# VIDILabs/instantvnr

Hardware: AMD Instinct MI355X
Metric: fps at 1024^2 on 1024^3 volume (higher is better)
Workload: dtype f16

## Files before the change

include/vnr_amd.h:

```cpp
#ifndef VNR_AMD_H
#define VNR_AMD_H

#include <stddef.h>
#include <stdint.h>

#ifdef __cplusplus
extern "C" {
#endif

#define VNR_AMD_OK 0
#define VNR_AMD_ERROR 1

typedef struct vnrAmdVolume_t*           vnrAmdVolume;
typedef struct vnrAmdRenderer_t*         vnrAmdRenderer;
typedef struct vnrAmdTransferFunction_t* vnrAmdTransferFunction;
typedef struct vnrAmdCamera_t*           vnrAmdCamera;

enum {
  VNR_AMD_OPTIX_NO_SHADING = 0,
  VNR_AMD_RAYMARCHING_NO_SHADING_DECODING = 4,
  VNR_AMD_RAYMARCHING_NO_SHADING_SAMPLE_STREAMING = 5,
  VNR_AMD_RAYMARCHING_NO_SHADING_IN_SHADER = 6,
  VNR_AMD_RAYMARCHING_GRADIENT_SHADING_SAMPLE_STREAMING = 8,
  VNR_AMD_RAYMARCHING_SINGLE_SHADE_HEURISTIC_SAMPLE_STREAMING = 11,
// ... 185 lines not shown
void vnrAmdReleaseVolume(vnrAmdVolume);

vnrAmdRenderer vnrAmdCreateRenderer(vnrAmdVolume);
int  vnrAmdRendererSetFramebufferSize(vnrAmdRenderer, int width, int height);
int  vnrAmdRendererSetTransferFunction(vnrAmdRenderer, vnrAmdTransferFunction);
int  vnrAmdRendererSetCamera(vnrAmdRenderer, vnrAmdCamera);
int  vnrAmdRendererSetMode(vnrAmdRenderer, int mode);
int  vnrAmdRendererSetDenoiser(vnrAmdRenderer, int enable);
int  vnrAmdRendererSetVolumeSamplingRate(vnrAmdRenderer, float rate);
int  vnrAmdRendererSetVolumeDensityScale(vnrAmdRenderer, float scale);
int  vnrAmdRendererResetAccumulation(vnrAmdRenderer);
int  vnrAmdRender(vnrAmdRenderer);
const float* vnrAmdRendererMapFrame(vnrAmdRenderer);
int  vnrAmdRendererSetOutputAsDeviceFramebuffer(vnrAmdRenderer, int enable);
int  vnrAmdRendererSetPixelRange(vnrAmdRenderer, uint32_t pixel_lo, uint32_t pixel_hi);
int  vnrAmdRendererSetPixelInterleave(vnrAmdRenderer, uint32_t block_pixels, uint32_t n_parts, uint32_t part);

typedef struct {
  uint64_t n_samples;
  uint64_t n_reference_slots;
  uint32_t n_iterations;
  uint32_t n_rays_hit;
  double   infer_kernel_ms;
  uint64_t infer_kernel_launches;
  double   infer_union_ms;
} vnrAmdFrameStats;
int  vnrAmdRendererGetFrameStats(vnrAmdRenderer, vnrAmdFrameStats*);
int  vnrAmdRendererSetProfiling(vnrAmdRenderer, int enable);
int  vnrAmdRendererSetAsync(vnrAmdRenderer, int enable);
int  vnrAmdRendererSetInShaderKernel(vnrAmdRenderer, int mode);
int  vnrAmdRendererDebugQueues(vnrAmdRenderer, const float** d_coords, const uint32_t** d_counters, float* iteration_ms, int max_iterations);
int  vnrAmdRendererDebugSchedule(vnrAmdRenderer, int out[4]);
int  vnrAmdDebugRaySourceIndex(const uint32_t* counts, uint32_t n_in, uint32_t* src_out, uint32_t* alive_out);
void vnrAmdReleaseRenderer(vnrAmdRenderer);

int  vnrAmdDistGetUniqueId(void* out128);
int  vnrAmdDistInit(int rank, int world_size, int local_rank, const void* unique_id, const char* transport, const char* address);
int  vnrAmdDistInitFromEnv(void);
int  vnrAmdDistFinalize(void);
int  vnrAmdDistRank(void);
int  vnrAmdDistWorldSize(void);
const char* vnrAmdDistTransport(void);
int  vnrAmdDistRcclRanksSeen(void);
int  vnrAmdDistBarrier(void);
int  vnrAmdDistAllReduceHost(double* values, int n, int op);
int  vnrAmdDistAllReduce(void* buf, size_t count, int dtype, int op);
int  vnrAmdDistAllGather(const void* send, void* recv, size_t bytes_per_rank);
int  vnrAmdDistReduceScatter(void* buf, size_t count_per_rank, int dtype);
int  vnrAmdDistBroadcast(void* buf, size_t bytes, int root);
int  vnrAmdDistSelfTest(double deadline_s, char* report, size_t report_size);
int  vnrAmdRendererSetDistributed(vnrAmdRenderer, int enable);
const float* vnrAmdRendererGatherFrame(vnrAmdRenderer);
int  vnrAmdRendererRenderPipelined(vnrAmdRenderer, const float** previous_frame);
int  vnrAmdRendererGetCompletedFrameStats(vnrAmdRenderer, vnrAmdFrameStats*);
int  vnrAmdRendererFlushPipeline(vnrAmdRenderer, const float** last_frame);
int  vnrAmdNeuralVolumeTrainDataParallel(vnrAmdVolume, int steps, int fast_mode);
int  vnrAmdNeuralVolumeSyncReplicas(vnrAmdVolume);
int  vnrAmdNeuralVolumeAllReduceGradients(vnrAmdVolume);
int  vnrAmdNeuralVolumeTrainEndDataParallel(vnrAmdVolume, int fast_mode, int sharded);
int  vnrAmdNeuralVolumeSetGradients(vnrAmdVolume, const float* host, size_t count);

int  vnrAmdMarchingCube(vnrAmdVolume, float isovalue, float** xyz, size_t* n_vertices, int on_device);
int  vnrAmdSaveTriangles(const char* filename, const float* xyz, size_t n_vertices);

void vnrAmdMemoryQuery(size_t* used_by_renderer, size_t* used_by_network);
void vnrAmdFreeTemporaryGPUMemory(void);
// ... 19 lines not shown
```

instantvnr_amd/_lib.py:

```python
import ctypes as C
import os
import re
import subprocess
import sys

_HERE = os.path.dirname(os.path.abspath(__file__))
ROOT = os.path.dirname(_HERE)
SO_PATH = os.environ.get("VNR_AMD_LIB_PATH") or os.path.join(_HERE, "libvnr_amd.so")
HEADER = os.path.join(ROOT, "include", "vnr_amd.h")

_lib = None
_torch_imported_before_load = None


class VnrAmdError(RuntimeError):
    pass


def require_torch_loaded_first():
    if _lib is not None and not _torch_imported_before_load:
        raise VnrAmdError("libvnr_amd.so was loaded before `import torch`: PyTorch's bundled ROCm runtime cannot share the "
                          "GPU with the system runtime the library already initialised.  Import torch first (instantvnr_amd."
                          "dist.init_from_env does when WORLD_SIZE > 1; tests/conftest.py does for the test session).")

# ... 148 lines not shown
    sig("vnrAmdNeuralVolumeSetInitSeed", I, P, U64)
    sig("vnrAmdVolumeSetClippingBox", I, P, FP, FP)
    sig("vnrAmdVolumeSetScaling", I, P, FP)
    sig("vnrAmdVolumeSetTransform", I, P, FP)
    sig("vnrAmdSimpleVolumeGetDataRange", I, P, FP)
    sig("vnrAmdMarchingCube", I, P, F, C.POINTER(C.POINTER(C.c_float)), C.POINTER(SZ), I)
    sig("vnrAmdSaveTriangles", I, C.c_char_p, C.POINTER(C.c_float), SZ)
    sig("vnrAmdVolumeGetValueRange", I, P, FP)
    sig("vnrAmdVolumeGetDims", I, P, IP)
    sig("vnrAmdVolumeIsNetwork", I, P)
    sig("vnrAmdVolumeGetMacrocell", I, P, IP, FP, C.POINTER(P), C.POINTER(P))
    sig("vnrAmdReleaseVolume", None, P)
    sig("vnrAmdCreateRenderer", P, P)
    sig("vnrAmdRendererSetFramebufferSize", I, P, I, I)
    sig("vnrAmdRendererSetTransferFunction", I, P, P)
    sig("vnrAmdRendererSetCamera", I, P, P)
    sig("vnrAmdRendererSetMode", I, P, I)
    sig("vnrAmdRendererSetDenoiser", I, P, I)
    sig("vnrAmdRendererSetVolumeSamplingRate", I, P, F)
    sig("vnrAmdRendererSetVolumeDensityScale", I, P, F)
    sig("vnrAmdRendererResetAccumulation", I, P)
    sig("vnrAmdRender", I, P)
    sig("vnrAmdRendererMapFrame", P, P)
    sig("vnrAmdRendererSetOutputAsDeviceFramebuffer", I, P, I)
    sig("vnrAmdRendererSetPixelRange", I, P, U32, U32)
    sig("vnrAmdRendererSetPixelInterleave", I, P, U32, U32, U32)
    sig("vnrAmdRendererGetFrameStats", I, P, C.POINTER(FrameStats))
    sig("vnrAmdRendererSetProfiling", I, P, I)
    sig("vnrAmdRendererSetAsync", I, P, I)
    sig("vnrAmdRendererSetInShaderKernel", I, P, I)
    sig("vnrAmdRendererDebugQueues", I, P, C.POINTER(P), C.POINTER(P), FP, I)
    sig("vnrAmdRendererDebugSchedule", I, P, IP)
    sig("vnrAmdDebugRaySourceIndex", I, P, U32, P, C.POINTER(U32))
    sig("vnrAmdReleaseRenderer", None, P)
    sig("vnrAmdDistGetUniqueId", I, P)
    sig("vnrAmdDistInit", I, I, I, I, P, C.c_char_p, C.c_char_p)
    sig("vnrAmdDistInitFromEnv", I)
    sig("vnrAmdDistFinalize", I)
    sig("vnrAmdDistRank", I)
    sig("vnrAmdDistWorldSize", I)
    sig("vnrAmdDistTransport", C.c_char_p)
    sig("vnrAmdDistRcclRanksSeen", I)
    sig("vnrAmdDistBarrier", I)
    sig("vnrAmdDistAllReduceHost", I, C.POINTER(D), I, I)
    sig("vnrAmdDistAllReduce", I, P, SZ, I, I)
    sig("vnrAmdDistAllGather", I, P, P, SZ)
    sig("vnrAmdDistReduceScatter", I, P, SZ, I)
    sig("vnrAmdDistBroadcast", I, P, SZ, I)
    sig("vnrAmdDistSelfTest", I, C.c_double, C.c_char_p, SZ)
    sig("vnrAmdRendererSetDistributed", I, P, I)
    sig("vnrAmdRendererGatherFrame", P, P)
    sig("vnrAmdRendererRenderPipelined", I, P, C.POINTER(P))
    sig("vnrAmdRendererGetCompletedFrameStats", I, P, C.POINTER(FrameStats))
    sig("vnrAmdRendererFlushPipeline", I, P, C.POINTER(P))
    sig("vnrAmdNeuralVolumeTrainDataParallel", I, P, I, I)
    sig("vnrAmdNeuralVolumeSyncReplicas", I, P)
    sig("vnrAmdNeuralVolumeSetBrickImageMode", I, P, I)
    sig("vnrAmdNeuralVolumeSetBrickImageBudget", I, P, SZ)
    sig("vnrAmdNeuralVolumeBrickImageLevels", C.c_uint, P)
    sig("vnrAmdNeuralVolumeGridBackwardPlan", I, P, U64, C.POINTER(U32), C.POINTER(U64))
    sig("vnrAmdNeuralVolumeSetDeterministicTraining", I, P, I)
    sig("vnrAmdNeuralVolumeGetDeterministicTraining", I, P, C.POINTER(I))
    sig("vnrAmdNeuralVolumeBrickImagePolicy", I, P, C.POINTER(U64), C.POINTER(C.c_uint), IP, C.POINTER(U64))
    sig("vnrAmdNeuralVolumeSetTrainProfiling", I, P, I)
    sig("vnrAmdNeuralVolumeGetTrainProfile", I, P, C.POINTER(D), IP)
    sig("vnrAmdNeuralVolumeAllReduceGradients", I, P)
# ... 57 lines not shown
```

instantvnr_amd/api.py:

```python
import ctypes as C
import json

import numpy as np

from . import _lib
from ._lib import VnrAmdError, check, check_ptr, lib

JSON_TEXT, JSON_BSON, JSON_TEXT_FILE, JSON_BSON_FILE = 0, 1, 2, 3

VALUE_TYPES = {np.dtype(np.uint8): 0, np.dtype(np.int8): 1, np.dtype(np.uint16): 2, np.dtype(np.int16): 3,
               np.dtype(np.uint32): 4, np.dtype(np.int32): 5, np.dtype(np.float32): 8, np.dtype(np.float64): 12}


def _fp(a):
    return a.ctypes.data_as(C.POINTER(C.c_float))


def _vec(v, n=3):
    a = np.ascontiguousarray(v, dtype=np.float32).ravel()
    assert a.size == n
    return a


def _json_arg(j, params=False):
# ... 708 lines not shown

def vnrRendererSetOutputAsDeviceFramebuffer(r, flag):
    check(lib().vnrAmdRendererSetOutputAsDeviceFramebuffer(r.h, 1 if flag else 0))
    r._device_output = bool(flag)


def vnrRendererSetProfiling(r, flag):
    check(lib().vnrAmdRendererSetProfiling(r.h, 1 if flag else 0))


def vnrRendererGetFrameStats(r):
    s = _lib.FrameStats()
    check(lib().vnrAmdRendererGetFrameStats(r.h, C.byref(s)))
    return {k: getattr(s, k) for k, _ in s._fields_}


def renderer_schedule(r):
    out = (C.c_int * 4)()
    check(lib().vnrAmdRendererDebugSchedule(r.h, out))
    return {"n_iters": out[0], "n_parts": out[1], "fused_pack": bool(out[2]), "decoupled": bool(out[3])}


def ray_source_index(counts, n_in):
    n_in = int(n_in)
    counts = np.ascontiguousarray(counts, dtype=np.uint32)
    if n_in <= 0 or counts.shape != ((n_in + 63) // 64,):
        raise ValueError("counts must hold one entry per 64-ray group of n_in > 0 rays")
    src = np.zeros(n_in, dtype=np.uint32)
    alive = C.c_uint32()
    check(lib().vnrAmdDebugRaySourceIndex(counts.ctypes.data, n_in, src.ctypes.data, C.byref(alive)))
    return src[:alive.value].copy(), int(alive.value)


def neural_brick_image(v):
    u, b, ms = C.c_int(), C.c_size_t(), C.c_float()
    check(lib().vnrAmdNeuralVolumeBrickImageInfo(v.h, C.byref(u), C.byref(b), C.byref(ms)))
    builds, after, tier, small = C.c_uint64(), C.c_uint(), C.c_int(), C.c_uint64()
    check(lib().vnrAmdNeuralVolumeBrickImagePolicy(v.h, C.byref(builds), C.byref(after), C.byref(tier), C.byref(small)))
    return {"in_use": bool(u.value), "bytes": b.value, "build_ms": ms.value, "levels": int(lib().vnrAmdNeuralVolumeBrickImageLevels(v.h)),
            "builds": int(builds.value), "launches_before_next_build": int(after.value), "tier": int(tier.value), "small_builds": int(small.value)}


def neural_set_brick_budget(v, n_bytes):
    check(lib().vnrAmdNeuralVolumeSetBrickImageBudget(v.h, int(n_bytes)))


def neural_info(v):
    vals = [C.c_int() for _ in range(5)]
    n = C.c_uint64()
    check(lib().vnrAmdNeuralVolumeGetInfo(v.h, *[C.byref(x) for x in vals], C.byref(n)))
    keys = ["n_levels", "n_features_per_level", "padded_width", "n_neurons", "n_hidden_layers"]
    d = {k: x.value for k, x in zip(keys, vals)}
    d["n_params"] = n.value
    kind = [C.c_int() for _ in range(6)]
    check(lib().vnrAmdNeuralVolumeGetModelKind(v.h, *[C.byref(x) for x in kind]))
    d.update({k: x.value for k, x in zip(["activation", "output_activation", "grid_type", "interpolation", "mfma_kernels", "mfma_training_kernels"], kind)})
    return d


def neural_grid_backward_plan(v, batch=65536):
    u32, u64 = (C.c_uint32 * 4)(), (C.c_uint64 * 2)()
    check(lib().vnrAmdNeuralVolumeGridBackwardPlan(v.h, int(batch), u32, u64))
    return {"n_levels": u32[0], "lds_levels": u32[1], "tile_entries": u32[2], "lds_blocks": u32[3], "atomic_requests": int(u64[0]), "flush_requests_at_most": int(u64[1])}


def neural_set_deterministic_training(v, enable=True):
# ... 183 lines not shown
```

instantvnr_amd/csrc/capi.cpp:

```cpp
#include "../../include/vnr_amd.h"

#include <cstdlib>
#include <cstdio>
#include <fstream>
#include <limits>
#include <memory>

#include "correction_budget.h"
#include "dist.h"
#include "renderer.h"
#include "scene.h"

using namespace vnr;

struct vnrAmdVolume_t { std::shared_ptr<VolumeBase> v; };
struct vnrAmdRenderer_t { std::unique_ptr<Renderer> r; std::shared_ptr<VolumeBase> volume; };
struct vnrAmdTransferFunction_t { TransferFunctionData d; };
struct vnrAmdCamera_t { CameraData d; };
struct vnrAmdCorrection_t { std::shared_ptr<Correction> c; };

namespace {
thread_local std::string g_last_error;

template <typename F>
// ... 988 lines not shown
}
int vnrAmdRendererGetFrameStats(vnrAmdRenderer r, vnrAmdFrameStats* s)
{
  return guarded([&]() {
    VNR_REN(r);
    const FrameStats& f = r->r->stats();
    s->n_samples = f.n_samples; s->n_reference_slots = f.n_reference_slots; s->n_iterations = f.n_iterations;
    s->n_rays_hit = f.n_rays_hit; s->infer_kernel_ms = f.infer_kernel_ms; s->infer_kernel_launches = f.infer_kernel_launches; s->infer_union_ms = f.infer_union_ms;
  });
}
int vnrAmdRendererDebugQueues(vnrAmdRenderer r, const float** d_coords, const uint32_t** d_counters, float* iteration_ms, int max_iterations)
{
  return guarded([&]() {
    VNR_REN(r);
    if (d_coords) *d_coords = r->r->debug_coords();
    if (d_counters) *d_counters = r->r->debug_counters();
    const auto& v = r->r->debug_iteration_ms();
    for (int i = 0; i < max_iterations; ++i) iteration_ms[i] = i < (int)v.size() ? v[i] : 0.0f;
  });
}
int vnrAmdRendererDebugSchedule(vnrAmdRenderer r, int out[4])
{
  return guarded([&]() {
    VNR_REN(r);
    if (!out) throw std::runtime_error("null output");
    const int* v = r->r->debug_schedule();
    for (int i = 0; i < 4; ++i) out[i] = v[i];
  });
}
int vnrAmdDebugRaySourceIndex(const uint32_t* counts, uint32_t n_in, uint32_t* src_out, uint32_t* alive_out)
{
  return guarded([&]() { debug_ray_source_index(counts, n_in, src_out, alive_out); });
}
int vnrAmdRendererSetProfiling(vnrAmdRenderer r, int e) { return guarded([&]() { VNR_REN(r); r->r->set_profiling(e != 0); }); }
int vnrAmdRendererSetAsync(vnrAmdRenderer r, int e) { return guarded([&]() { VNR_REN(r); r->r->set_async(e != 0); }); }
int vnrAmdRendererSetInShaderKernel(vnrAmdRenderer r, int m) { return guarded([&]() { VNR_REN(r); r->r->set_in_shader_kernel(m); }); }
void vnrAmdReleaseRenderer(vnrAmdRenderer r) { delete r; }

int vnrAmdDistGetUniqueId(void* out128) { return guarded([&]() { if (!out128) throw std::runtime_error("null id buffer"); rccl_unique_id(out128); }); }
static void bind_device_to_local_rank(int local_rank)
{
  const int count = vnrAmdDeviceCount();
  if (count > 0) Runtime::get().init(local_rank % count);
}
int vnrAmdDistInit(int rank, int world, int local_rank, const void* unique_id, const char* transport, const char* address)
{
  return guarded([&]() {
    bind_device_to_local_rank(local_rank);
    Dist::get().init(rank, world, local_rank, unique_id, transport, address ? address : "");
  });
}
int vnrAmdDistInitFromEnv(void)
{
  return guarded([&]() {
    const char* lr = std::getenv("LOCAL_RANK");
    const char* r = std::getenv("RANK");
    bind_device_to_local_rank(lr && *lr ? std::atoi(lr) : (r && *r ? std::atoi(r) : 0));
    Dist::get().init_from_env();
  });
}
int vnrAmdDistFinalize(void) { return guarded([&]() { Dist::get().finalize(); }); }
int vnrAmdDistRank(void) { return Dist::get().rank(); }
int vnrAmdDistWorldSize(void) { return Dist::get().world(); }
const char* vnrAmdDistTransport(void) { return Dist::get().transport_name(); }
int vnrAmdDistRcclRanksSeen(void) { return Dist::get().rccl_ranks_seen(); }
int vnrAmdDistBarrier(void)
// ... 220 lines not shown
```

instantvnr_amd/csrc/infer_kernel.h:

```cpp
#pragma once
#include <algorithm>
#include <cstdlib>

#include "infer_tile.h"
#include "pack_rays.h"

namespace vnr {

struct FusedMlp {
  const uint16_t* packed;
  uint32_t lds_halves, width, n_hidden_matmuls, activation, output_activation;
  bool general;
  bool weights_global;
  float quantize_threshold;
};

struct InferArgs {
  const LevelInfo* levels;
  uint32_t n_levels, interpolation;
  const half_t* table;
  uint32_t table_bytes;
  const uint8_t* brick_image;
  const half_t* packed_mlp;
  const float* coords;
  float* out;
  half_t* features_out;
  half_t* acts_out;
  const uint32_t* n_ptr;
  const uint32_t* dest;
  uint32_t queue_mode;
  uint32_t out_stride;
  uint32_t n;
  uint32_t n_hidden_matmuls;
  uint32_t activation;
  uint32_t output_activation;
  uint32_t lds_halves;
  uint32_t sharers;
  uint32_t weights_global;
  float quantize_threshold;
  PackArgs pack;
};

template <int F, int K_IN, int W, int MODE, bool GENERAL>
__global__ void __launch_bounds__(64 * MlpShape<W>::WAVES) fused_infer_kernel(const InferArgs args)
{
  constexpr int NCHUNK = K_IN / 8;
  constexpr uint32_t WAVES = MlpShape<W>::WAVES;
  extern __shared__ __attribute__((aligned(16))) half_t lds[];

  const uint32_t lane = threadIdx.x & 63u;
  const uint32_t wave = threadIdx.x >> 6;

  if (MODE == 0 && WAVES == 4 && args.pack.n_blocks) {
    uint32_t* s_part = (uint32_t*)lds;
    for (uint32_t item = blockIdx.x; item < args.pack.n_blocks; item += gridDim.x) {
      pack_rays_block<4>(args.pack, item, s_part);
      __syncthreads();
    }
  }
  const uint32_t n = args.n_ptr ? min(*args.n_ptr, args.n) : args.n;
  const uint32_t n_tiles = (n + 63u) >> 6;
  const uint32_t xcd = blockIdx.x & 7u;
  const uint32_t per_xcd = (n_tiles + 7u) >> 3;
  const uint32_t waves_per_xcd = (gridDim.x >> 3) * WAVES;
  const uint32_t tile_end = min(n_tiles, (xcd + 1u) * per_xcd);
  if (xcd * per_xcd + (blockIdx.x >> 3) * WAVES >= tile_end) return;

  constexpr bool CAN_GLOBAL = GENERAL;
  const bool wglobal = CAN_GLOBAL && args.weights_global != 0u;
  if (MODE != 1 && !wglobal) {
    const uint4_t* src = (const uint4_t*)args.packed_mlp;
    uint4_t* dst = (uint4_t*)lds;
    for (uint32_t i = threadIdx.x; i < args.lds_halves / 8; i += blockDim.x) dst[i] = src[i];
    __syncthreads();
  }
  const uint32_t nh = args.n_hidden_matmuls;
  const uint32_t act = args.activation;
  const uint32_t h = lane >> 5;
  const uint32_t r = lane & 31u;
  const table_rsrc_t rsrc = make_table_rsrc(args.table, args.table_bytes);

  for (uint32_t tile = xcd * per_xcd + (blockIdx.x >> 3) * WAVES + wave; tile < tile_end; tile += waves_per_xcd) {
    const uint32_t i = tile * 64u + lane;
    const uint32_t ic = min(i, n - 1u);
    float3_packed p;
    uint32_t out_index = i;
    if (args.queue_mode) {
      const uint4_t rec = ((const uint4_t*)args.coords)[ic];
      p = {__uint_as_float(rec.x), __uint_as_float(rec.y), __uint_as_float(rec.z)};
      out_index = rec.w * args.out_stride;
    } else {
      p = ((const float3_packed*)args.coords)[ic];
      if (args.dest) out_index = args.dest[ic];
    }

    half8_t feat[NCHUNK];
    encode_tile<F, K_IN, GENERAL>(args.levels, args.n_levels, args.interpolation, rsrc, args.brick_image, p.x, p.y, p.z, feat,
                                  GENERAL ? args.quantize_threshold : 0.0f);

    if (MODE != 0 && args.features_out && i < n) {
      half8_t* dst = (half8_t*)(args.features_out + (size_t)i * K_IN);
#pragma unroll
      for (int c = 0; c < NCHUNK; ++c) dst[c] = feat[c];
    }
    if (MODE == 1) continue;

    float y;
    if (CAN_GLOBAL && wglobal)
      y = mlp_tile<W, K_IN, MODE == 2, GENERAL>(args.packed_mlp, feat, nh, act, h, r, args.acts_out, n, tile * 64u);
    else
      y = mlp_tile<W, K_IN, MODE == 2, GENERAL>((const half_t*)lds, feat, nh, act, h, r, args.acts_out, n, tile * 64u);
    if (i < n) args.out[out_index] = finish_output<GENERAL>(y, args.output_activation);
  }
}

template <int F, int K_IN, int W, int MODE, bool GENERAL>
static void launch_one(const InferArgs& a, size_t n_max, hipStream_t s)
{
  constexpr uint32_t WAVES = MlpShape<W>::WAVES;
  const Runtime& rt = Runtime::get();
  const uint32_t n_tiles = div_round_up(n_max, 64);
  uint32_t blocks = div_round_up(n_tiles, WAVES);
  static const uint32_t forced = [] {
    const char* e = std::getenv("VNR_AMD_INFER_BLOCKS_PER_CU");
    const int v = e ? std::atoi(e) : 0;
    return (uint32_t)(v >= 1 && v <= 64 ? v : 0);
  }();
  const size_t shmem = (MODE == 1 || a.weights_global) ? 16 : (size_t)a.lds_halves * sizeof(uint16_t);
  const uint32_t fit = (uint32_t)std::max<size_t>(1, std::min<size_t>(4, (160 * 1024) / std::max<size_t>(shmem, 1)));
  uint32_t max_blocks = (uint32_t)rt.n_cus * (forced ? forced : std::min(fit, a.sharers >= 2 ? 3u : 4u));
  if (!forced && a.n_ptr && a.queue_mode) max_blocks = std::min((uint32_t)rt.n_cus * 32u, std::max((uint32_t)rt.n_cus * 4u, n_tiles / 33u));
  if (blocks > max_blocks) blocks = max_blocks;
  blocks = next_multiple(blocks, 8);
  auto kernel = fused_infer_kernel<F, K_IN, W, MODE, GENERAL>;
  static bool attr_set = false;
  if (!attr_set) {
    VNR_HIP_CHECK(hipFuncSetAttribute((const void*)kernel, hipFuncAttributeMaxDynamicSharedMemorySize, 160 * 1024));
    attr_set = true;
  }
  kernel<<<blocks, 64 * WAVES, shmem, s>>>(a);
  VNR_HIP_CHECK(hipGetLastError());
}

template <int W, int MODE, bool GENERAL>
static void dispatch(uint32_t F, uint32_t K_IN, const InferArgs& a, size_t n_max, hipStream_t s)
{
#define VNR_CASE(f, k) if (F == f && K_IN == k) return launch_one<f, k, W, MODE, GENERAL>(a, n_max, s)
  VNR_CASE(1, 16); VNR_CASE(1, 32);
  VNR_CASE(2, 16); VNR_CASE(2, 32); VNR_CASE(2, 48); VNR_CASE(2, 64);
  VNR_CASE(4, 16); VNR_CASE(4, 32); VNR_CASE(4, 48); VNR_CASE(4, 64); VNR_CASE(4, 80); VNR_CASE(4, 96); VNR_CASE(4, 112); VNR_CASE(4, 128);
  VNR_CASE(8, 16); VNR_CASE(8, 32); VNR_CASE(8, 48); VNR_CASE(8, 64); VNR_CASE(8, 80); VNR_CASE(8, 96); VNR_CASE(8, 112); VNR_CASE(8, 128);
#undef VNR_CASE
  throw std::runtime_error("unsupported encoding shape: n_features_per_level=" + std::to_string(F) +
                           " padded width=" + std::to_string(K_IN));
}

#define VNR_DEFINE_FUSED_WIDTH(W, GENERAL, SUFFIX)                                                                        \
  void launch_fused_w##W##SUFFIX(int mode, uint32_t F, uint32_t K_IN, const InferArgs& a, size_t n_max, hipStream_t s)    \
  {                                                                                                                       \
    if (mode == 0) dispatch<W, 0, GENERAL>(F, K_IN, a, n_max, s);                                                         \
    else dispatch<W, 2, GENERAL>(F, K_IN, a, n_max, s);                                                                   \
  }

}
```

instantvnr_amd/csrc/infer_tile.h:

```cpp
#pragma once
#include "grid_device.h"

namespace vnr {

struct float3_packed { float x, y, z; };

template <int W> struct MlpShape {
  static_assert(W == 16 || W == 32 || W == 64 || W == 128, "FullyFusedMLP widths");
  static constexpr int MT = W >= 32 ? W / 32 : 1;
  static constexpr int RW = 32 * MT;
  static constexpr int KS = W / 16;
  static constexpr int STEP = 16 * RW;
  static constexpr int HIDDEN = KS * STEP;
  static constexpr int LAST = KS * 16;
  static constexpr int WAVES = W == 128 ? 8 : 4;
};
__host__ __device__ inline uint32_t mlp_rows_padded(uint32_t W) { return W >= 32u ? W : 32u; }
__host__ __device__ inline uint32_t packed_mlp_halves(uint32_t in_width, uint32_t W, uint32_t n_hidden_matmuls)
{
  const uint32_t step = 16u * mlp_rows_padded(W);
  return (in_width / 16u) * step + n_hidden_matmuls * (W / 16u) * step + (W / 16u) * 16u;
}

__host__ __device__ inline uint32_t packedT_halves(uint32_t in_width, uint32_t W, uint32_t nh)
// ... 99 lines not shown
    for (int e = 0; e < 16; ++e) acc[m][e] = 0.0f;
#pragma unroll
  for (int s = 0; s < S1; ++s) {
#pragma unroll
    for (int m = 0; m < MT; ++m) {
      const half8_t a = *(const half8_t*)(wgt + ((s * 2 + h) * RW + m * 32 + r) * 8);
      acc[m] = __builtin_amdgcn_mfma_f32_32x32x16_f16(a, b1[s], acc[m], 0, 0, 0);
    }
  }
  half8_t bf[KS];
#pragma unroll
  for (int s = 0; s < KS; ++s) bf[s] = pack_act<GENERAL>(acc[s >> 1], s & 1, act);
  if (TRAIN && acts_out && smp_ok) store_acts<KS>(acts_out + (size_t)smp * W, bf, h);

  for (uint32_t layer = 0; layer < nh; ++layer) {
    const half_t* w = wgt + S1 * Sh::STEP + layer * Sh::HIDDEN;
#pragma unroll
    for (int m = 0; m < MT; ++m)
#pragma unroll
      for (int e = 0; e < 16; ++e) acc[m][e] = 0.0f;
#pragma unroll
    for (int s = 0; s < KS; ++s) {
#pragma unroll
      for (int m = 0; m < MT; ++m) {
        const half8_t a = *(const half8_t*)(w + ((s * 2 + h) * RW + m * 32 + r) * 8);
        acc[m] = __builtin_amdgcn_mfma_f32_32x32x16_f16(a, bf[s], acc[m], 0, 0, 0);
      }
    }
#pragma unroll
    for (int s = 0; s < KS; ++s) bf[s] = pack_act<GENERAL>(acc[s >> 1], s & 1, act);
    if (TRAIN && acts_out && smp_ok) store_acts<KS>(acts_out + ((size_t)(layer + 1) * n + smp) * W, bf, h);
  }

  const half_t* wl = wgt + S1 * Sh::STEP + nh * Sh::HIDDEN;
  float part = 0.0f;
#pragma unroll
  for (int s = 0; s < KS; ++s) {
    const half8_t wv = *(const half8_t*)(wl + (s * 2 + h) * 8);
#pragma unroll
    for (int q = 0; q < 4; ++q) {
      const half2_t a2 = {bf[s][2 * q], bf[s][2 * q + 1]};
      const half2_t w2 = {wv[2 * q], wv[2 * q + 1]};
      part = __builtin_amdgcn_fdot2(a2, w2, part, false);
    }
  }
  return part;
}



template <int F, int K_IN, bool GENERAL = false>
__device__ __forceinline__ void encode_tile(const LevelInfo* levels, uint32_t n_levels, uint32_t interpolation, const table_rsrc_t& rsrc,
                                            const uint8_t* brick_image, float x, float y, float z, half8_t (&feat)[K_IN / 8],
                                            float quantize_threshold = 0.0f)
{
  constexpr int L_PAD = K_IN / F;
  typedef const __attribute__((address_space(4))) LevelInfo* const_levels_t;
  const LevelInfo* lvtab_generic = levels;
  asm volatile("" : "+s"(lvtab_generic));
  const const_levels_t lvtab = (const_levels_t)lvtab_generic;
  auto level_consts = [&](int l) {
    LevelInfo lv;
    lv.scale = __builtin_bit_cast(float, __builtin_amdgcn_readfirstlane(__builtin_bit_cast(int, lvtab[l].scale)));
    lv.resolution = __builtin_amdgcn_readfirstlane(lvtab[l].resolution);
    lv.res2 = __builtin_amdgcn_readfirstlane(lvtab[l].res2);
    lv.size = __builtin_amdgcn_readfirstlane(lvtab[l].size);
    lv.offset = __builtin_amdgcn_readfirstlane(lvtab[l].offset);
    lv.hashed = __builtin_amdgcn_readfirstlane(lvtab[l].hashed);
    lv.brick = __builtin_amdgcn_readfirstlane(lvtab[l].brick);
    lv.pad1 = __builtin_amdgcn_readfirstlane(lvtab[l].pad1);
    return lv;
  };
#pragma unroll
  for (int l = 0; l < L_PAD; ++l) {
    half_t o[F];
#pragma unroll
    for (int f = 0; f < F; ++f) o[f] = (half_t)0.0f;
    if (l < (int)n_levels) encode_level_fast<F, GENERAL>(level_consts(l), interpolation, rsrc, brick_image, x, y, z, o, quantize_threshold);
#pragma unroll
    for (int f = 0; f < F; ++f) feat[(l * F + f) / 8][(l * F + f) % 8] = o[f];
    if ((l & 3) == 3) __builtin_amdgcn_sched_barrier(0);
  }
}

template <int W, int K_IN, bool TRAIN, bool GENERAL = false>
__device__ __forceinline__ float mlp_tile(const half_t* __restrict__ wgt, half8_t (&feat)[K_IN / 8], uint32_t nh, uint32_t act, uint32_t h,
                                          uint32_t r, half_t* acts_out, size_t n, uint32_t tile_base)
{
  constexpr int S1 = K_IN / 16;
#pragma unroll
  for (int s = 0; s < S1; ++s) swap_halves8(feat[2 * s], feat[2 * s + 1]);

  float part[2];
#pragma unroll
  for (int nt = 0; nt < 2; ++nt) {
    half8_t b1[S1];
#pragma unroll
    for (int s = 0; s < S1; ++s) b1[s] = feat[2 * s + nt];
    const uint32_t smp = tile_base + 32u * nt + r;
    part[nt] = mlp_column_tile<W, S1, TRAIN, GENERAL>(wgt, b1, nh, act, h, r, acts_out, n, smp, smp < n);
  }

  uint32_t p0 = __builtin_bit_cast(uint32_t, part[0]), p1 = __builtin_bit_cast(uint32_t, part[1]);
  swap_halves(p0, p1);
  return __builtin_bit_cast(float, p0) + __builtin_bit_cast(float, p1);
}

template <bool GENERAL = false>
__device__ __forceinline__ float finish_output(float y, uint32_t out_act)
{
  if (!GENERAL) return (float)(half_t)y;
  return (float)act_forward_f16((half_t)y, out_act);
}

struct TileNet {
// ... 24 lines not shown
```

instantvnr_amd/csrc/network.h:

```cpp
#pragma once

#include <functional>
#include <utility>
#include <vector>

#include "common.h"
#include "json.h"

namespace vnr {

constexpr int kMaxLevels = 32;
constexpr size_t kLdsBytes = 160 * 1024;
constexpr int kLossScale = 128;

struct LevelInfo {
  float scale;
  uint32_t resolution;
  uint32_t res2;
  uint32_t size;
  uint32_t offset;
  uint32_t hashed;
  uint32_t brick;
  uint32_t pad1;
};
// ... 175 lines not shown
  mutable DeviceBuffer<LevelInfo> levels_brick_dev_{MemTag::Network};
  mutable bool brick_valid_ = false, brick_refused_ = false;
  mutable uint32_t brick_stable_calls_ = 0;
  static constexpr uint32_t kBrickPaysAfter = 64;
  mutable uint32_t brick_served_calls_ = 0, brick_after_scale_ = 1;
  mutable uint64_t brick_builds_ = 0;
  static constexpr size_t kBrickSmallMinLaunch = (size_t)1 << 20;
  mutable int brick_tier_ = 0;
  mutable bool brick_small_refused_ = false;
  mutable uint64_t brick_small_builds_ = 0;
  mutable float brick_build_ms_ = 0.0f;
  uint32_t brick_res_cap_ = 0;
  size_t brick_budget_ = 0;
  mutable uint32_t brick_levels_mask_ = 0;
  int brick_mode_ = -1;

public:
  static constexpr int kTrainPhases = 5, kTrainProfileSteps = 64;
  void set_train_profiling(bool e);
  int train_profile(double* ms_per_step );
private:
  void profile_mark(int phase_boundary, hipStream_t s);
  bool train_profiling_ = false;
  std::vector<hipEvent_t> prof_events_;
  uint64_t prof_steps_ = 0;

public:
  ~Network();
  Network(const Network&) = delete;
  Network& operator=(const Network&) = delete;
};

uint32_t grid_make_layout(const ModelConfig& cfg, GridDevice* out);

}
```

instantvnr_amd/csrc/network_infer.hip:

```cpp
#include "infer_kernel.h"

namespace vnr {

__global__ void pack_mlp_kernel(const half_t* __restrict__ params, half_t* __restrict__ packed, half_t* __restrict__ packedT, uint32_t in_width,
                                uint32_t W, uint32_t nh)
{
  const uint32_t RW = mlp_rows_padded(W), KS = W / 16u, step = 16u * RW, hidden = KS * step;
  const uint32_t total = packed_mlp_halves(in_width, W, nh), totalT = packedT ? packedT_halves(in_width, W, nh) : 0u;
  const uint32_t l1 = (in_width / 16u) * step;
  const uint32_t first_sz = W * in_width;
  for (uint32_t e = blockIdx.x * blockDim.x + threadIdx.x; e < total + totalT; e += gridDim.x * blockDim.x) {
    half_t v = (half_t)0.0f;
    if (e < total) {
      if (e < l1) {
        const uint32_t j = e & 7u, q = e >> 3, row = q % RW, hs = q / RW, h = hs & 1u, s = hs >> 1;
        if (row < W) v = params[row * in_width + 16u * s + 8u * h + j];
      } else if (e < l1 + nh * hidden) {
        const uint32_t r = e - l1, layer = r / hidden, qq = r % hidden;
        const uint32_t j = qq & 7u, q = qq >> 3, row = q % RW, hs = q / RW, h = hs & 1u, s = hs >> 1;
        const uint32_t k = 16u * s + 8u * (j >> 2) + 4u * h + (j & 3u);
        if (row < W) v = params[first_sz + layer * W * W + row * W + k];
      } else {
        const uint32_t q = e - l1 - nh * hidden;
        const uint32_t j = q & 7u, h = (q >> 3) & 1u, s = q >> 4;
// ... 3 lines not shown
      packed[e] = v;
    } else {
      const uint32_t t = e - total;
      const uint32_t rp = ((in_width + 31u) / 32u) * 32u;
      if (t < KS * 16u) {
        const uint32_t j = t & 7u, h = (t >> 3) & 1u, s = t >> 4;
        v = params[first_sz + nh * W * W + 16u * s + 8u * (j >> 2) + 4u * h + (j & 3u)];
      } else if (t < KS * 16u + nh * hidden) {
        const uint32_t r = t - KS * 16u, layer = r / hidden, qq = r % hidden;
        const uint32_t j = qq & 7u, q = qq >> 3, row = q % RW, hs = q / RW, h = hs & 1u, s = hs >> 1;
        const uint32_t kk = 16u * s + 8u * (j >> 2) + 4u * h + (j & 3u);
        if (row < W) v = params[first_sz + layer * W * W + kk * W + row];
      } else {
        const uint32_t qq = t - KS * 16u - nh * hidden;
        const uint32_t j = qq & 7u, q = qq >> 3, row = q % rp, hs = q / rp, h = hs & 1u, s = hs >> 1;
        const uint32_t kk = 16u * s + 8u * (j >> 2) + 4u * h + (j & 3u);
        if (row < in_width) v = params[kk * in_width + row];
      }
      packedT[t] = v;
    }
  }
}

void launch_pack_mlp(const uint16_t* params, uint16_t* packed, uint16_t* packedT, uint32_t in_width, uint32_t W, uint32_t n_hidden_matmuls, hipStream_t s)
{
  const uint32_t total = packed_mlp_halves(in_width, W, n_hidden_matmuls) + (packedT ? packedT_halves(in_width, W, n_hidden_matmuls) : 0u);
  pack_mlp_kernel<<<div_round_up(total, 256), 256, 0, s>>>((const half_t*)params, (half_t*)packed, (half_t*)packedT, in_width, W, n_hidden_matmuls);
}

#define VNR_DECL(name) void name(int mode, uint32_t F, uint32_t K_IN, const InferArgs& a, size_t n_max, hipStream_t s)
VNR_DECL(launch_fused_w16); VNR_DECL(launch_fused_w32); VNR_DECL(launch_fused_w64); VNR_DECL(launch_fused_w128);
VNR_DECL(launch_fused_w16g); VNR_DECL(launch_fused_w32g); VNR_DECL(launch_fused_w64g); VNR_DECL(launch_fused_w128g);
#undef VNR_DECL

void launch_fused(int mode, const GridDevice& grid, uint32_t in_width, const FusedMlp& mlp, const LevelInfo* d_levels, const uint16_t* table, size_t table_bytes,
                  const float* coords, float* out, uint16_t* features_out, uint16_t* acts_out, size_t n, const uint32_t* d_n, size_t n_max, hipStream_t s,
                  const uint32_t* d_dest, uint32_t queue_out_stride, const uint8_t* brick_image, uint32_t sharers, const PackArgs* pack)
{
  if (n_max == 0) { if (pack && pack->n_blocks) throw std::runtime_error("internal: ray packing fused into an empty evaluation launch"); return; }
  if (n_max > 0xffffffc0ull) throw std::runtime_error("inference batch too large (max 2^32-64 samples per call)");
  if (table_bytes >= (1ull << 32)) throw std::runtime_error("hash table >= 4 GiB is not supported");
  InferArgs a;
  a.levels = d_levels;
  a.n_levels = grid.n_levels;
  a.interpolation = grid.interpolation;
  a.table = (const half_t*)table;
  a.table_bytes = (uint32_t)table_bytes;
  a.brick_image = brick_image;
  a.sharers = sharers;
  a.packed_mlp = (const half_t*)mlp.packed;
  a.coords = coords;
  a.out = out;
  a.features_out = (half_t*)features_out;
  a.acts_out = (half_t*)acts_out;
  a.n_ptr = d_n;
  a.dest = d_dest;
  a.queue_mode = queue_out_stride ? 1u : 0u;
  a.out_stride = queue_out_stride;
  a.n = d_n ? (uint32_t)n_max : (uint32_t)n;
  a.n_hidden_matmuls = mlp.n_hidden_matmuls;
  a.activation = mlp.activation;
  a.output_activation = mlp.output_activation;
  a.lds_halves = mlp.lds_halves;
  a.weights_global = mlp.weights_global ? 1u : 0u;
  a.quantize_threshold = mlp.quantize_threshold;
  if (mlp.weights_global && !mlp.general) throw std::runtime_error("internal: weights from global memory are a GENERAL instance's");
// ... 20 lines not shown
```

Before: 279.6.

## Trim register pressure in fused inference kernel and size occupancy from register count

For the inference-only fast path, the output index is recomputed after the MLP instead of being held across the encoding, which shortens register live ranges. Encoding can be split into two unrolled level groups, and a scheduling barrier is added before the output layer. The launcher now queries the kernel's register count to work out how many blocks fit per CU, and with a brick image it allows 4–5 blocks per CU instead of 3–4. A debug API exposes the kernel's register, scratch and LDS usage. The risks are an extra global load of the queue record per sample and possible cache contention at the higher occupancy.

```diff
diff --git a/include/vnr_amd.h b/include/vnr_amd.h
--- a/include/vnr_amd.h
+++ b/include/vnr_amd.h
@@ -241,6 +241,7 @@
 int  vnrAmdRendererDebugQueues(vnrAmdRenderer, const float** d_coords, const uint32_t** d_counters, float* iteration_ms, int max_iterations);
 int  vnrAmdRendererDebugSchedule(vnrAmdRenderer, int out[4]);
 int  vnrAmdDebugRaySourceIndex(const uint32_t* counts, uint32_t n_in, uint32_t* src_out, uint32_t* alive_out);
+int  vnrAmdDebugEvalKernelResources(uint32_t F, uint32_t K_IN, uint32_t W, int general, int* regs, int* scratch_bytes, int* lds_bytes);
 void vnrAmdReleaseRenderer(vnrAmdRenderer);
 
 int  vnrAmdDistGetUniqueId(void* out128);
diff --git a/instantvnr_amd/_lib.py b/instantvnr_amd/_lib.py
--- a/instantvnr_amd/_lib.py
+++ b/instantvnr_amd/_lib.py
@@ -204,6 +204,7 @@
     sig("vnrAmdRendererDebugQueues", I, P, C.POINTER(P), C.POINTER(P), FP, I)
     sig("vnrAmdRendererDebugSchedule", I, P, IP)
     sig("vnrAmdDebugRaySourceIndex", I, P, U32, P, C.POINTER(U32))
+    sig("vnrAmdDebugEvalKernelResources", I, U32, U32, U32, I, IP, IP, IP)
     sig("vnrAmdReleaseRenderer", None, P)
     sig("vnrAmdDistGetUniqueId", I, P)
     sig("vnrAmdDistInit", I, I, I, I, P, C.c_char_p, C.c_char_p)
diff --git a/instantvnr_amd/api.py b/instantvnr_amd/api.py
--- a/instantvnr_amd/api.py
+++ b/instantvnr_amd/api.py
@@ -764,6 +764,13 @@
     return src[:alive.value].copy(), int(alive.value)
 
 
+def eval_kernel_resources(n_features, padded_width, n_neurons, general=False):
+    regs, scratch, lds = C.c_int(), C.c_int(), C.c_int()
+    check(lib().vnrAmdDebugEvalKernelResources(int(n_features), int(padded_width), int(n_neurons), int(bool(general)),
+                                               C.byref(regs), C.byref(scratch), C.byref(lds)))
+    return {"regs": regs.value, "scratch_bytes": scratch.value, "lds_bytes": lds.value}
+
+
 def neural_brick_image(v):
     u, b, ms = C.c_int(), C.c_size_t(), C.c_float()
     check(lib().vnrAmdNeuralVolumeBrickImageInfo(v.h, C.byref(u), C.byref(b), C.byref(ms)))
diff --git a/instantvnr_amd/csrc/capi.cpp b/instantvnr_amd/csrc/capi.cpp
--- a/instantvnr_amd/csrc/capi.cpp
+++ b/instantvnr_amd/csrc/capi.cpp
@@ -1044,6 +1044,10 @@
 {
   return guarded([&]() { debug_ray_source_index(counts, n_in, src_out, alive_out); });
 }
+int vnrAmdDebugEvalKernelResources(uint32_t F, uint32_t K_IN, uint32_t W, int general, int* regs, int* scratch_bytes, int* lds_bytes)
+{
+  return guarded([&]() { eval_kernel_resources(F, K_IN, W, general != 0, regs, scratch_bytes, lds_bytes); });
+}
 int vnrAmdRendererSetProfiling(vnrAmdRenderer r, int e) { return guarded([&]() { VNR_REN(r); r->r->set_profiling(e != 0); }); }
 int vnrAmdRendererSetAsync(vnrAmdRenderer r, int e) { return guarded([&]() { VNR_REN(r); r->r->set_async(e != 0); }); }
 int vnrAmdRendererSetInShaderKernel(vnrAmdRenderer r, int m) { return guarded([&]() { VNR_REN(r); r->r->set_in_shader_kernel(m); }); }
diff --git a/instantvnr_amd/csrc/infer_kernel.h b/instantvnr_amd/csrc/infer_kernel.h
--- a/instantvnr_amd/csrc/infer_kernel.h
+++ b/instantvnr_amd/csrc/infer_kernel.h
@@ -46,6 +46,7 @@
 {
   constexpr int NCHUNK = K_IN / 8;
   constexpr uint32_t WAVES = MlpShape<W>::WAVES;
+  constexpr bool DIET = MODE == 0 && !GENERAL;
   extern __shared__ __attribute__((aligned(16))) half_t lds[];
 
   const uint32_t lane = threadIdx.x & 63u;
@@ -88,14 +89,14 @@
     if (args.queue_mode) {
       const uint4_t rec = ((const uint4_t*)args.coords)[ic];
       p = {__uint_as_float(rec.x), __uint_as_float(rec.y), __uint_as_float(rec.z)};
-      out_index = rec.w * args.out_stride;
+      if (!DIET) out_index = rec.w * args.out_stride;
     } else {
       p = ((const float3_packed*)args.coords)[ic];
       if (args.dest) out_index = args.dest[ic];
     }
 
     half8_t feat[NCHUNK];
-    encode_tile<F, K_IN, GENERAL>(args.levels, args.n_levels, args.interpolation, rsrc, args.brick_image, p.x, p.y, p.z, feat,
+    encode_tile<F, K_IN, GENERAL, DIET>(args.levels, args.n_levels, args.interpolation, rsrc, args.brick_image, p.x, p.y, p.z, feat,
                                   GENERAL ? args.quantize_threshold : 0.0f);
 
     if (MODE != 0 && args.features_out && i < n) {
@@ -110,9 +111,18 @@
       y = mlp_tile<W, K_IN, MODE == 2, GENERAL>(args.packed_mlp, feat, nh, act, h, r, args.acts_out, n, tile * 64u);
     else
       y = mlp_tile<W, K_IN, MODE == 2, GENERAL>((const half_t*)lds, feat, nh, act, h, r, args.acts_out, n, tile * 64u);
-    if (i < n) args.out[out_index] = finish_output<GENERAL>(y, args.output_activation);
+    if (DIET) {
+      uint32_t tile_again = tile;
+      asm volatile("" : "+v"(tile_again));
+      const uint32_t j = tile_again * 64u + lane;
+      if (args.queue_mode) out_index = ((const uint32_t*)args.coords)[(size_t)min(j, n - 1u) * 4u + 3u] * args.out_stride;
+      else if (!args.dest) out_index = j;
+      if (j < n) args.out[out_index] = finish_output<GENERAL>(y, args.output_activation);
+    } else if (i < n) args.out[out_index] = finish_output<GENERAL>(y, args.output_activation);
   }
 }
+
+constexpr uint32_t kBlocksPerCuAlone = 5, kBlocksPerCuShared = 4;
 
 template <int F, int K_IN, int W, int MODE, bool GENERAL>
 static void launch_one(const InferArgs& a, size_t n_max, hipStream_t s)
@@ -127,12 +137,19 @@
     return (uint32_t)(v >= 1 && v <= 64 ? v : 0);
   }();
   const size_t shmem = (MODE == 1 || a.weights_global) ? 16 : (size_t)a.lds_halves * sizeof(uint16_t);
-  const uint32_t fit = (uint32_t)std::max<size_t>(1, std::min<size_t>(4, (160 * 1024) / std::max<size_t>(shmem, 1)));
-  uint32_t max_blocks = (uint32_t)rt.n_cus * (forced ? forced : std::min(fit, a.sharers >= 2 ? 3u : 4u));
+  auto kernel = fused_infer_kernel<F, K_IN, W, MODE, GENERAL>;
+  static const uint32_t fit_regs = [&] {
+    hipFuncAttributes at{};
+    VNR_HIP_CHECK(hipFuncGetAttributes(&at, (const void*)kernel));
+    const uint32_t waves = std::min(8u, 512u / std::max(8u, next_multiple((uint32_t)at.numRegs, 8u)));
+    return MODE == 0 ? std::max(4u, waves * 4u / WAVES) : 4u;
+  }();
+  const uint32_t fit = (uint32_t)std::max<size_t>(1, std::min<size_t>(fit_regs, (160 * 1024) / std::max<size_t>(shmem, 1)));
+  const uint32_t policy = a.brick_image ? (a.sharers >= 2 ? kBlocksPerCuShared : kBlocksPerCuAlone) : (a.sharers >= 2 ? 3u : 4u);
+  uint32_t max_blocks = (uint32_t)rt.n_cus * (forced ? forced : std::min(fit, policy));
   if (!forced && a.n_ptr && a.queue_mode) max_blocks = std::min((uint32_t)rt.n_cus * 32u, std::max((uint32_t)rt.n_cus * 4u, n_tiles / 33u));
   if (blocks > max_blocks) blocks = max_blocks;
   blocks = next_multiple(blocks, 8);
-  auto kernel = fused_infer_kernel<F, K_IN, W, MODE, GENERAL>;
   static bool attr_set = false;
   if (!attr_set) {
     VNR_HIP_CHECK(hipFuncSetAttribute((const void*)kernel, hipFuncAttributeMaxDynamicSharedMemorySize, 160 * 1024));
@@ -142,17 +159,33 @@
   VNR_HIP_CHECK(hipGetLastError());
 }
 
+#define VNR_ENCODING_SHAPES(X)                                                                                  \
+  X(1, 16) X(1, 32)                                                                                             \
+  X(2, 16) X(2, 32) X(2, 48) X(2, 64)                                                                           \
+  X(4, 16) X(4, 32) X(4, 48) X(4, 64) X(4, 80) X(4, 96) X(4, 112) X(4, 128)                                     \
+  X(8, 16) X(8, 32) X(8, 48) X(8, 64) X(8, 80) X(8, 96) X(8, 112) X(8, 128)
+
+[[noreturn]] static void unsupported_shape(uint32_t F, uint32_t K_IN)
+{
+  throw std::runtime_error("unsupported encoding shape: n_features_per_level=" + std::to_string(F) + " padded width=" + std::to_string(K_IN));
+}
+
 template <int W, int MODE, bool GENERAL>
 static void dispatch(uint32_t F, uint32_t K_IN, const InferArgs& a, size_t n_max, hipStream_t s)
 {
-#define VNR_CASE(f, k) if (F == f && K_IN == k) return launch_one<f, k, W, MODE, GENERAL>(a, n_max, s)
-  VNR_CASE(1, 16); VNR_CASE(1, 32);
-  VNR_CASE(2, 16); VNR_CASE(2, 32); VNR_CASE(2, 48); VNR_CASE(2, 64);
-  VNR_CASE(4, 16); VNR_CASE(4, 32); VNR_CASE(4, 48); VNR_CASE(4, 64); VNR_CASE(4, 80); VNR_CASE(4, 96); VNR_CASE(4, 112); VNR_CASE(4, 128);
-  VNR_CASE(8, 16); VNR_CASE(8, 32); VNR_CASE(8, 48); VNR_CASE(8, 64); VNR_CASE(8, 80); VNR_CASE(8, 96); VNR_CASE(8, 112); VNR_CASE(8, 128);
+#define VNR_CASE(f, k) if (F == f && K_IN == k) return launch_one<f, k, W, MODE, GENERAL>(a, n_max, s);
+  VNR_ENCODING_SHAPES(VNR_CASE)
 #undef VNR_CASE
-  throw std::runtime_error("unsupported encoding shape: n_features_per_level=" + std::to_string(F) +
-                           " padded width=" + std::to_string(K_IN));
+  unsupported_shape(F, K_IN);
+}
+
+template <int W, int MODE, bool GENERAL>
+static void dispatch_attributes(uint32_t F, uint32_t K_IN, hipFuncAttributes* out)
+{
+#define VNR_CASE(f, k) if (F == f && K_IN == k) { VNR_HIP_CHECK(hipFuncGetAttributes(out, (const void*)fused_infer_kernel<f, k, W, MODE, GENERAL>)); return; }
+  VNR_ENCODING_SHAPES(VNR_CASE)
+#undef VNR_CASE
+  unsupported_shape(F, K_IN);
 }
 
 #define VNR_DEFINE_FUSED_WIDTH(W, GENERAL, SUFFIX)                                                                        \
@@ -160,6 +193,7 @@
   {                                                                                                                       \
     if (mode == 0) dispatch<W, 0, GENERAL>(F, K_IN, a, n_max, s);                                                         \
     else dispatch<W, 2, GENERAL>(F, K_IN, a, n_max, s);                                                                   \
-  }
+  }                                                                                                                       \
+  void fused_attributes_w##W##SUFFIX(uint32_t F, uint32_t K_IN, hipFuncAttributes* out) { dispatch_attributes<W, 0, GENERAL>(F, K_IN, out); }
 
 }
diff --git a/instantvnr_amd/csrc/infer_tile.h b/instantvnr_amd/csrc/infer_tile.h
--- a/instantvnr_amd/csrc/infer_tile.h
+++ b/instantvnr_amd/csrc/infer_tile.h
@@ -155,6 +155,7 @@
     if (TRAIN && acts_out && smp_ok) store_acts<KS>(acts_out + ((size_t)(layer + 1) * n + smp) * W, bf, h);
   }
 
+  if (!GENERAL) __builtin_amdgcn_sched_barrier(0);
   const half_t* wl = wgt + S1 * Sh::STEP + nh * Sh::HIDDEN;
   float part = 0.0f;
 #pragma unroll
@@ -172,7 +173,7 @@
 
 
 
-template <int F, int K_IN, bool GENERAL = false>
+template <int F, int K_IN, bool GENERAL = false, bool SPLIT = false>
 __device__ __forceinline__ void encode_tile(const LevelInfo* levels, uint32_t n_levels, uint32_t interpolation, const table_rsrc_t& rsrc,
                                             const uint8_t* brick_image, float x, float y, float z, half8_t (&feat)[K_IN / 8],
                                             float quantize_threshold = 0.0f)
@@ -182,6 +183,7 @@
   const LevelInfo* lvtab_generic = levels;
   asm volatile("" : "+s"(lvtab_generic));
   const const_levels_t lvtab = (const_levels_t)lvtab_generic;
+  if (!GENERAL) asm volatile("" : "+s"(n_levels));
   auto level_consts = [&](int l) {
     LevelInfo lv;
     lv.scale = __builtin_bit_cast(float, __builtin_amdgcn_readfirstlane(__builtin_bit_cast(int, lvtab[l].scale)));
@@ -194,16 +196,24 @@
     lv.pad1 = __builtin_amdgcn_readfirstlane(lvtab[l].pad1);
     return lv;
   };
-#pragma unroll
-  for (int l = 0; l < L_PAD; ++l) {
-    half_t o[F];
-#pragma unroll
-    for (int f = 0; f < F; ++f) o[f] = (half_t)0.0f;
-    if (l < (int)n_levels) encode_level_fast<F, GENERAL>(level_consts(l), interpolation, rsrc, brick_image, x, y, z, o, quantize_threshold);
-#pragma unroll
-    for (int f = 0; f < F; ++f) feat[(l * F + f) / 8][(l * F + f) % 8] = o[f];
-    if ((l & 3) == 3) __builtin_amdgcn_sched_barrier(0);
-  }
+#define VNR_ENCODE_ONE_LEVEL(l)                                                                                                              \
+  {                                                                                                                                          \
+    half_t o[F];                                                                                                                             \
+    _Pragma("unroll") for (int f = 0; f < F; ++f) o[f] = (half_t)0.0f;                                                                       \
+    if (l < (int)n_levels) encode_level_fast<F, GENERAL>(level_consts(l), interpolation, rsrc, brick_image, x, y, z, o, quantize_threshold); \
+    _Pragma("unroll") for (int f = 0; f < F; ++f) feat[(l * F + f) / 8][(l * F + f) % 8] = o[f];                                             \
+    if ((l & 3) == 3) __builtin_amdgcn_sched_barrier(0);                                                                                     \
+  }
+  if constexpr (SPLIT && L_PAD > 16) {
+#pragma unroll
+    for (int l = 0; l < 16; ++l) VNR_ENCODE_ONE_LEVEL(l)
+#pragma unroll
+    for (int l = 16; l < L_PAD; ++l) VNR_ENCODE_ONE_LEVEL(l)
+  } else {
+#pragma unroll
+    for (int l = 0; l < L_PAD; ++l) VNR_ENCODE_ONE_LEVEL(l)
+  }
+#undef VNR_ENCODE_ONE_LEVEL
 }
 
 template <int W, int K_IN, bool TRAIN, bool GENERAL = false>
diff --git a/instantvnr_amd/csrc/network.h b/instantvnr_amd/csrc/network.h
--- a/instantvnr_amd/csrc/network.h
+++ b/instantvnr_amd/csrc/network.h
@@ -231,5 +231,6 @@
 };
 
 uint32_t grid_make_layout(const ModelConfig& cfg, GridDevice* out);
+void eval_kernel_resources(uint32_t F, uint32_t K_IN, uint32_t W, bool general, int* regs, int* scratch_bytes, int* lds_bytes);
 
 }
diff --git a/instantvnr_amd/csrc/network_infer.hip b/instantvnr_amd/csrc/network_infer.hip
--- a/instantvnr_amd/csrc/network_infer.hip
+++ b/instantvnr_amd/csrc/network_infer.hip
@@ -59,6 +59,25 @@
 VNR_DECL(launch_fused_w16); VNR_DECL(launch_fused_w32); VNR_DECL(launch_fused_w64); VNR_DECL(launch_fused_w128);
 VNR_DECL(launch_fused_w16g); VNR_DECL(launch_fused_w32g); VNR_DECL(launch_fused_w64g); VNR_DECL(launch_fused_w128g);
 #undef VNR_DECL
+#define VNR_DECL(name) void name(uint32_t F, uint32_t K_IN, hipFuncAttributes* out)
+VNR_DECL(fused_attributes_w16); VNR_DECL(fused_attributes_w32); VNR_DECL(fused_attributes_w64); VNR_DECL(fused_attributes_w128);
+VNR_DECL(fused_attributes_w16g); VNR_DECL(fused_attributes_w32g); VNR_DECL(fused_attributes_w64g); VNR_DECL(fused_attributes_w128g);
+#undef VNR_DECL
+
+void eval_kernel_resources(uint32_t F, uint32_t K_IN, uint32_t W, bool general, int* regs, int* scratch_bytes, int* lds_bytes)
+{
+  hipFuncAttributes at{};
+  switch (W) {
+  case 16: general ? fused_attributes_w16g(F, K_IN, &at) : fused_attributes_w16(F, K_IN, &at); break;
+  case 32: general ? fused_attributes_w32g(F, K_IN, &at) : fused_attributes_w32(F, K_IN, &at); break;
+  case 64: general ? fused_attributes_w64g(F, K_IN, &at) : fused_attributes_w64(F, K_IN, &at); break;
+  case 128: general ? fused_attributes_w128g(F, K_IN, &at) : fused_attributes_w128(F, K_IN, &at); break;
+  default: throw std::runtime_error("no MFMA kernel for n_neurons = " + std::to_string(W));
+  }
+  if (regs) *regs = at.numRegs;
+  if (scratch_bytes) *scratch_bytes = (int)at.localSizeBytes;
+  if (lds_bytes) *lds_bytes = (int)at.sharedSizeBytes;
+}
 
 void launch_fused(int mode, const GridDevice& grid, uint32_t in_width, const FusedMlp& mlp, const LevelInfo* d_levels, const uint16_t* table, size_t table_bytes,
                   const float* coords, float* out, uint16_t* features_out, uint16_t* acts_out, size_t n, const uint32_t* d_n, size_t n_max, hipStream_t s,
```

After: 291.1, median of 6. 1.04x the previous value.
